# lorenzovaquero/BUSCA

Hardware: AMD Instinct MI355X
Metric: BUSCA association steps/sec (DT-step: features in HBM -> logits/probs/argmax), MOT17-like 32 lost x 16 proposals (higher is better)
Workload: dtype f32

## Files before the change

### busca_amd/csrc/busca_hip.hip

```cpp
#include "busca_internal.hpp"

#define BUSCA_DT_BUCKET_KERNEL 1
#include "dt_kernel.hip.inc"
#include "pairwise_kernel.hip.inc"
#include "track_kernel.hip.inc"
#include "crop_kernel.hip.inc"
#include "ecc_kernel.hip.inc"

int ensure_lds(busca_ctx* c, const void* kern, size_t bytes) {
    if (c->lds_configured.count(kern)) return BUSCA_OK;
    HIP_TRY(c, hipFuncSetAttribute(kern, hipFuncAttributeMaxDynamicSharedMemorySize, (int)bytes));
    c->lds_configured.insert(kern);
    return BUSCA_OK;
}

enum { OPT_INT , OPT_FLAG , OPT_PRESENT , OPT_READONLY  };
struct BuscaOptionDesc { const char* env; const char* opt; int BuscaOptions::*field; int kind; };
static const BuscaOptionDesc BUSCA_OPTIONS[] = {
    {"BUSCA_DT_NTRK", "dt_ntrk", &BuscaOptions::dt_ntrk, OPT_INT}, {"BUSCA_DT_TILED", "dt_tiled", &BuscaOptions::dt_tiled, OPT_PRESENT},
    {"BUSCA_DT_SPLIT", "dt_split", &BuscaOptions::dt_split, OPT_INT}, {"BUSCA_DT_PROF", nullptr, &BuscaOptions::dt_prof, OPT_INT},
    {"BUSCA_DT_PRUNE", "dt_prune", &BuscaOptions::dt_prune, OPT_INT}, {nullptr, "last_dt_prune", &BuscaOptions::last_dt_prune, OPT_READONLY},
    {"BUSCA_DTL_RT", nullptr, &BuscaOptions::dtl_rt, OPT_INT}, {"BUSCA_DTL_RT_MASK", nullptr, &BuscaOptions::dtl_rt_mask, OPT_INT},
    {"BUSCA_DTL_FFN", nullptr, &BuscaOptions::dtl_ffn, OPT_INT}, {"BUSCA_DTL_ATTN", nullptr, &BuscaOptions::dtl_attn, OPT_INT},
    {"BUSCA_CROP_BAND", "crop_band", &BuscaOptions::crop_band, OPT_INT}, {nullptr, "dt_exact_f32", &BuscaOptions::dt_exact_f32, OPT_FLAG},
    {nullptr, "last_dt_grid", &BuscaOptions::last_dt_grid, OPT_READONLY}, {nullptr, "last_dt_ntrk", &BuscaOptions::last_dt_ntrk, OPT_READONLY},
    {nullptr, "last_dt_split", &BuscaOptions::last_dt_split, OPT_READONLY},
    {"BUSCA_ASSIGN_STAGE", "assign_stage", &BuscaOptions::assign_stage, OPT_INT}, {nullptr, "last_assign_staged", &BuscaOptions::last_assign_staged, OPT_READONLY},
};
static const BuscaOptionDesc* option_by_name(const char* name) {
    for (const BuscaOptionDesc& e : BUSCA_OPTIONS) if (e.opt && !strcmp(e.opt, name)) return &e;
    return nullptr;
}
static void options_from_env(BuscaOptions& o) {
    for (const BuscaOptionDesc& e : BUSCA_OPTIONS)
        if (const char* t = e.env ? getenv(e.env) : nullptr) o.*e.field = e.kind == OPT_PRESENT ? 1 : atoi(t);
}

extern "C" int busca_version(void) { return 2002; }

static std::string g_create_err;

extern "C" int busca_ctx_create(int device, busca_ctx** out) {
    if (!out) return BUSCA_EINVAL;
    *out = nullptr;
    int n = 0;
    hipError_t e = hipGetDeviceCount(&n);
    if (e != hipSuccess || n <= 0) {
        g_create_err = std::string("hipGetDeviceCount: ") + hipGetErrorString(e) + ", devices=" + std::to_string(n);
        return BUSCA_EHIP;
    }
    if (device < 0 || device >= n) { g_create_err = "device index out of range"; return BUSCA_EINVAL; }
    e = hipSetDevice(device);
    if (e != hipSuccess) { g_create_err = std::string("hipSetDevice: ") + hipGetErrorString(e); return BUSCA_EHIP; }
    busca_ctx* c = new busca_ctx();
    c->device = device;
    options_from_env(c->opt);
    c->reid = reid_state_new();
    *out = c;
    return BUSCA_OK;
}

#ifndef BUSCA_BUILD_FLAGS
#define BUSCA_BUILD_FLAGS "unknown"
#endif
extern "C" const char* busca_build_info(void) { return "libbusca_hip gfx950 flags: " BUSCA_BUILD_FLAGS; }

extern "C" int busca_set_option(busca_ctx* c, const char* name, int32_t value) {
    if (!c || !name) return BUSCA_EINVAL;
    if (!strncmp(name, "reid_", 5)) return reid_set_option(c, name, value);
    if (!strcmp(name, "dt_status")) { if (c->dt.xerr) *c->dt.xerr = value; return BUSCA_OK; }
    const BuscaOptionDesc* e = option_by_name(name);
    if (!e || e->kind == OPT_READONLY) return fail(c, BUSCA_EINVAL, "busca_set_option: unknown option '%s'", name);
    c->opt.*e->field = e->kind == OPT_FLAG ? value != 0 : value;
    return BUSCA_OK;
}
extern "C" int busca_get_option(busca_ctx* c, const char* name, int32_t* value) {
    if (!c || !name || !value) return BUSCA_EINVAL;
    if (!strncmp(name, "reid_", 5)) return reid_get_option(c, name, value);
    if (!strcmp(name, "dt_status")) { *value = c->dt.xerr ? *c->dt.xerr : 0; return BUSCA_OK; }
    const BuscaOptionDesc* e = option_by_name(name);
    if (!e) return fail(c, BUSCA_EINVAL, "busca_get_option: unknown option '%s'", name);
    *value = c->opt.*e->field;
    return BUSCA_OK;
}

void timing_drain(busca_ctx* c) {
    for (auto& pr : c->ev_pending) {
        float ms = 0.f;
        if (hipEventSynchronize(pr.second) == hipSuccess && hipEventElapsedTime(&ms, pr.first, pr.second) == hipSuccess) {
            c->t_ms += ms;
            c->t_n += 1;
        }
        c->ev_free.push_back(pr.first);
        c->ev_free.push_back(pr.second);
    }
    c->ev_pending.clear();
}

extern "C" void busca_ctx_destroy(busca_ctx* c) {
    if (!c) return;
    hipSetDevice(c->device);
    hipDeviceSynchronize();
    timing_drain(c);
    for (auto e : c->ev_free) hipEventDestroy(e);
// ... 355 lines not shown
```

### busca_amd/csrc/busca_internal.hpp

```cpp
#pragma once
#include <hip/hip_runtime.h>
#include <hip/hip_fp16.h>

#include <algorithm>
#include <cmath>
#include <cstdarg>
#include <cstdio>
#include <cstdlib>
#include <cstring>
#include <set>
#include <string>
#include <type_traits>
#include <vector>

#pragma GCC visibility push(default)
#include "../../include/busca_hip.h"
#pragma GCC visibility pop
#include "dt_types.hpp"

struct ReidState;

struct DTTiledW {
    const void* w_embed = nullptr;
    const void *w_in[DT_MAX_LAYERS] = {}, *w_out[DT_MAX_LAYERS] = {}, *w1[DT_MAX_LAYERS] = {}, *w2[DT_MAX_LAYERS] = {};
};

struct DTState {
    bool loaded = false;
    busca_dt_cfg cfg{};
    void* dev_blob = nullptr;
    size_t dev_bytes = 0;
    DTParams proto{};
    void* dev_blob32 = nullptr;
    DTParams proto32{};
    void* dev_tiled = nullptr;
    DTTiledW tw;
    void* ws = nullptr; size_t ws_bytes = 0;
    void* xch = nullptr; unsigned* xflag = nullptr; float* xlg = nullptr; int* xerr = nullptr; int* xerr_dev = nullptr; int xslots = 0; unsigned xepoch = 0;
    int num_cu = 256;
};

struct BuscaOptions {
    int dt_ntrk = 0;
    int dt_tiled = 0;
    int dtl_rt = 0;
    int dtl_rt_mask = -1;
    int dtl_ffn = 2;
    int dtl_attn = 1;
    int dt_split = -1;
    int dt_prune = -1;
    int dt_prof = 0;
    int dt_exact_f32 = 0;
    int crop_band = 1;
    int assign_stage = -1;
    int last_assign_staged = 0;
    int last_dt_grid = 0, last_dt_ntrk = 0, last_dt_split = 0;
    int last_dt_prune = 0;
};

struct busca_ctx {
    int device = 0;
    std::string err;
    BuscaOptions opt;
    DTState dt;
    ReidState* reid = nullptr;
    bool timing = false;
    std::vector<std::pair<hipEvent_t, hipEvent_t>> ev_pending;
    std::vector<hipEvent_t> ev_free;
    double t_ms = 0.0;
    long long t_n = 0;
    int* crop_fill = nullptr;
    int crop_fill_cap = 0;
    std::set<const void*> lds_configured;
    void* ecc_ws = nullptr; size_t ecc_ws_bytes = 0;
};

int ensure_lds(busca_ctx* c, const void* kern, size_t bytes);

static inline int fail(busca_ctx* c, int code, const char* fmt, ...) {
    char buf[512];
    va_list ap;
    va_start(ap, fmt);
    vsnprintf(buf, sizeof buf, fmt, ap);
    va_end(ap);
    if (c) c->err = buf;
    return code;
}
#define HIP_TRY(c, call)                                                                                   \
    do {                                                                                                   \
        hipError_t e__ = (call);                                                                           \
        if (e__ != hipSuccess) return fail((c), BUSCA_EHIP, "%s -> %s", #call, hipGetErrorString(e__));     \
    } while (0)


void timing_drain(busca_ctx* c);
hipEvent_t timing_event(busca_ctx* c);
struct TimedLaunch {
    busca_ctx* c; hipStream_t s; hipEvent_t e0{}, e1{}; bool on;
    TimedLaunch(busca_ctx* c_, hipStream_t s_) : c(c_), s(s_), on(c_->timing) {
        if (on) { e0 = timing_event(c); e1 = timing_event(c); hipEventRecord(e0, s); }
    }
    ~TimedLaunch() {
        if (on) { hipEventRecord(e1, s); c->ev_pending.emplace_back(e0, e1); if (c->ev_pending.size() > 4096) timing_drain(c); }
    }
};

#define BUSCA_ENOKERNEL 1000
int dt_fused_f32(busca_ctx* c, const DTParams& K, int MT, int d, hipStream_t s);
int dt_fused_f16(busca_ctx* c, const DTParams& K, int MT, int d, bool two, hipStream_t s);
int dt_fused_x3(busca_ctx* c, const DTParams& K, int MT, int d, hipStream_t s);
int dt_tiled_f32(busca_ctx* c, const DTParams& K, int d, hipStream_t s);
int dt_tiled_f16(busca_ctx* c, const DTParams& K, int d, hipStream_t s);
int dt_tiled_x3(busca_ctx* c, const DTParams& K, int d, hipStream_t s);
int dt_split_ensure(busca_ctx* c);
size_t dtl_ws_bytes(size_t M, int D, int FF, size_t es);
int dtl_ws_ensure(busca_ctx* c, size_t need, hipStream_t s);
void dt_bucket_ids_launch(busca_ctx* c, hipStream_t s, const float* mem_ltrb, const float* can_ltrb, int B, int L, int P, int fake_f64, int can_pos, int nspec, int sep_can, int* ids);
ReidState* reid_state_new();
void reid_state_delete(ReidState* r);
bool reid_state_loaded(const ReidState* r);
int reid_set_option(busca_ctx* c, const char* name, int32_t value);
int reid_get_option(busca_ctx* c, const char* name, int32_t* value);
```

### busca_amd/csrc/dt_kernel.hip.inc

```

#pragma clang fp contract(off)

#include "dt_types.hpp"

static __device__ __forceinline__ float dt_fma(float a, float b, float c) { return __builtin_fmaf(a, b, c); }
static __device__ __forceinline__ f32x4 dt_fma(f32x4 a, f32x4 b, f32x4 c) { return __builtin_elementwise_fma(a, b, c); }

#define DT_STAMP(slot) do { if (p.prof != nullptr && blockIdx.x == 0 && lane == 0) p.prof[wave * DT_PROF_SLOTS + (slot)] = (long long)__builtin_readcyclecounter(); } while (0)

template <int PREC> struct Prec;
template <> struct Prec<0> {
    typedef float elem;
    typedef u32x4 op_t;
    static constexpr int ES = 4, EP = 4, CHUNK = 16, SUB = 4, CW = 64;
    static __device__ __forceinline__ op_t wload(const u32x4* __restrict__ w) { return *w; }
    static __device__ __forceinline__ op_t xload(const char* p, int) { return *(const u32x4*)p; }
    static __device__ __forceinline__ f32x4 unscale(f32x4 v) { return v; }
    static __device__ __forceinline__ f32x4 prescale(f32x4 v) { return v; }
    static __device__ __forceinline__ void mma(f32x4& acc, u32x4 a, u32x4 b) {
        f32x4 af = __builtin_bit_cast(f32x4, a), bf = __builtin_bit_cast(f32x4, b);
        acc = __builtin_amdgcn_mfma_f32_16x16x4f32(af[0], bf[0], acc, 0, 0, 0);
        acc = __builtin_amdgcn_mfma_f32_16x16x4f32(af[1], bf[1], acc, 0, 0, 0);
        acc = __builtin_amdgcn_mfma_f32_16x16x4f32(af[2], bf[2], acc, 0, 0, 0);
        acc = __builtin_amdgcn_mfma_f32_16x16x4f32(af[3], bf[3], acc, 0, 0, 0);
// ... 26 lines not shown
        h16x8 h;
        f32x4 lo = t[2 * c];
        f32x4 hi = (2 * c + 1 < NT) ? t[(2 * c + 1 < NT) ? 2 * c + 1 : 0] : (f32x4){0.f, 0.f, 0.f, 0.f};
#pragma unroll
        for (int r = 0; r < 4; ++r) { h[r] = (_Float16)lo[r]; h[4 + r] = (_Float16)hi[r]; }
        return __builtin_bit_cast(u32x4, h);
    }
    static __device__ __forceinline__ bool store4(char* p, f32x4 v, int = 0) {
        h16x4 h; h[0] = (_Float16)v[0]; h[1] = (_Float16)v[1]; h[2] = (_Float16)v[2]; h[3] = (_Float16)v[3];
        *(h16x4*)p = h;
        return false;
    }
    static __device__ __forceinline__ float exp(float x) { return __expf(x); }
    static __device__ __forceinline__ f32x4 gelu(f32x4 v) {
        const f32x4 s = v * 0.70710678118654752440f;
        f32x4 ax = __builtin_elementwise_min(__builtin_elementwise_abs(s), (f32x4){4.f, 4.f, 4.f, 4.f});
        auto k4 = [](float c) { return (f32x4){c, c, c, c}; };
        f32x4 q = dt_fma(ax, k4(-0.00014198364806361496f), k4(0.0036634085699915886f));
        q = dt_fma(q, ax, k4(-0.030893569812178612f));
        q = dt_fma(q, ax, k4(0.1496966928243637f));
        q = dt_fma(q, ax, k4(0.9181665182113647f));
        q = dt_fma(q, ax, k4(1.627924919128418f));
        const f32x4 m = q * -ax;
        f32x4 e;
#pragma unroll
        for (int r = 0; r < 4; ++r) e[r] = __builtin_amdgcn_exp2f(m[r]);
        f32x4 erf_ = 1.0f - e;
#pragma unroll
        for (int r = 0; r < 4; ++r) erf_[r] = __builtin_copysignf(erf_[r], s[r]);
        return (v * 0.5f) * (erf_ + 1.0f);
    }
};

struct X3Op { u32x4 hi, lo; };
typedef _Float16 dt_h16x2 __attribute__((ext_vector_type(2)));
typedef float dt_f32x2 __attribute__((ext_vector_type(2)));
static __device__ __forceinline__ void dt_split2(float t0, float t1, unsigned& hi, unsigned& lo) {
    const dt_h16x2 h = __builtin_convertvector((dt_f32x2){t0, t1}, dt_h16x2);
    hi = __builtin_bit_cast(unsigned, h);
    unsigned l;
    asm("v_fma_mixlo_f16 %0, %1, -1.0, %2 op_sel_hi:[1,0,0]" : "=v"(l) : "v"(hi), "v"(t0));
    asm("v_fma_mixhi_f16 %0, %1, -1.0, %2 op_sel:[1,0,0] op_sel_hi:[1,0,0]" : "+v"(l) : "v"(hi), "v"(t1));
    lo = l;
}
template <> struct Prec<2> {
    typedef _Float16 elem;
    typedef X3Op op_t;
    static constexpr int ES = 4, EP = 2, CHUNK = 32, SUB = 8, CW = 128;
    static __device__ __forceinline__ op_t wload(const u32x4* __restrict__ w) { op_t o; o.hi = w[0]; o.lo = w[64]; return o; }
    static __device__ __forceinline__ op_t xload(const char* p, int po) { op_t o; o.hi = *(const u32x4*)p; o.lo = *(const u32x4*)(p + po); return o; }
    static __device__ __forceinline__ void mma(f32x4& acc, op_t a, op_t b) {
        acc = __builtin_amdgcn_mfma_f32_16x16x32_f16(__builtin_bit_cast(h16x8, a.lo), __builtin_bit_cast(h16x8, b.hi), acc, 0, 0, 0);
        acc = __builtin_amdgcn_mfma_f32_16x16x32_f16(__builtin_bit_cast(h16x8, a.hi), __builtin_bit_cast(h16x8, b.lo), acc, 0, 0, 0);
        acc = __builtin_amdgcn_mfma_f32_16x16x32_f16(__builtin_bit_cast(h16x8, a.hi), __builtin_bit_cast(h16x8, b.hi), acc, 0, 0, 0);
    }
    static __device__ __forceinline__ f32x4 unscale(f32x4 v) { return v * (1.0f / (DT_X3_XS * DT_X3_WS)); }
    static __device__ __forceinline__ f32x4 prescale(f32x4 v) { return v * (DT_X3_XS * DT_X3_WS); }
    static __device__ __forceinline__ bool store4(char* p, f32x4 v, int po) {
        const f32x4 lim = {65504.f, 65504.f, 65504.f, 65504.f};
        const f32x4 sv = v * DT_X3_XS, av = __builtin_elementwise_abs(sv);
        const bool clipped = fmaxf(fmaxf(av[0], av[1]), fmaxf(av[2], av[3])) > 65504.f;
        const f32x4 s = __builtin_elementwise_min(__builtin_elementwise_max(sv, -lim), lim);
        unsigned h0, h1, l0, l1;
        dt_split2(s[0], s[1], h0, l0);
        dt_split2(s[2], s[3], h1, l1);
        *(u32x2*)p = (u32x2){h0, h1};
        *(u32x2*)(p + po) = (u32x2){l0, l1};
        return clipped;
    }
    static __device__ __forceinline__ float exp(float x) { return __expf(x); }
    static __device__ __forceinline__ f32x4 gelu(f32x4 v) { return Prec<0>::gelu(v); }
};
template <int PREC> struct AttPrec { typedef Prec<PREC == 2 ? 0 : PREC> type; };


template <int PREC, int NW, int PF, int WMAX>
__device__ __forceinline__ void gemm_prefetch(typename Prec<PREC>::op_t (&wf)[PF][WMAX], const u32x4* __restrict__ w, int tstride) {
#pragma unroll
    for (int p = 0; p < PF; ++p)
#pragma unroll
        for (int i = 0; i < NW; ++i) wf[p][i] = Prec<PREC>::wload(w + i * tstride + p * Prec<PREC>::CW);
}

template <int PREC, int NW, int NX, int NKC, int PF, bool W_IS_A, int NWN, int WMAX, int XM = 0>
__device__ __forceinline__ void gemm_stream(f32x4 (&acc)[NW][NX], typename Prec<PREC>::op_t (&wf)[PF][WMAX], const u32x4* __restrict__ w, int tstride,
                                            const char* lds, int RS, const u32x4* __restrict__ wn, int tstride_n) {
    static_assert(NKC % PF == 0 && NW <= WMAX && NWN <= WMAX && (XM != 1 || PF % 2 == 0), "bad streaming geometry");
    typedef Prec<PREC> PR;
    constexpr int CW = PR::CW;
    const int po = (RS - 16) / 2;
    typename PR::op_t xf[XM == 1 ? 2 : 1][NX];
    if constexpr (XM == 1) {
#pragma unroll
        for (int j = 0; j < NX; ++j) xf[0][j] = PR::xload(lds + j * 16 * RS, po);
    }
#pragma unroll 1
    for (int k0 = 0; k0 < NKC; k0 += PF) {
#pragma unroll
        for (int p = 0; p < PF; ++p) {
            const int kx = k0 + p + 1 < NKC ? k0 + p + 1 : NKC - 1;
            if constexpr (XM == 1) {
#pragma unroll
                for (int j = 0; j < NX; ++j) xf[(p + 1) & 1][j] = PR::xload(lds + j * 16 * RS + kx * 64, po);
                __builtin_amdgcn_sched_barrier(0);
            } else {
#pragma unroll
                for (int j = 0; j < NX; ++j) xf[0][j] = PR::xload(lds + j * 16 * RS + (k0 + p) * 64, po);
            }
            constexpr int XS = XM == 1 ? 1 : 0;
#pragma unroll
            for (int i = 0; i < NW; ++i)
#pragma unroll
                for (int j = 0; j < NX; ++j) {
                    if (W_IS_A) Prec<PREC>::mma(acc[i][j], wf[p][i], xf[p & XS][j]);
                    else        Prec<PREC>::mma(acc[i][j], xf[p & XS][j], wf[p][i]);
                }
            const int kn = k0 + p + PF;
            if (kn < NKC) {
#pragma unroll
                for (int i = 0; i < NW; ++i) wf[p][i] = PR::wload(w + i * tstride + kn * CW);
            } else if (NWN > 0) {
#pragma unroll
                for (int i = 0; i < NWN; ++i) wf[p][i] = PR::wload(wn + i * tstride_n + (kn - NKC) * CW);
            }
        }
    }
}

static __device__ __forceinline__ float xor_sum_b(float v) {
    v += __shfl_xor(v, 16);
    v += __shfl_xor(v, 32);
    return v;
}
static __device__ __forceinline__ float xor_max_b(float v) {
    v = fmaxf(v, __shfl_xor(v, 16));
    v = fmaxf(v, __shfl_xor(v, 32));
    return v;
}

template <typename R> static __device__ __forceinline__ R log_r(R x);
template <> __device__ __forceinline__ float log_r<float>(float x) { return (float)log((double)x); }
template <> __device__ __forceinline__ double log_r<double>(double x) { return log(x); }

template <typename R>
static __device__ __forceinline__ void bucket_xy_size(R x1, R y1, R x2, R y2, float rx1, float ry1, float rx2,
                                                      float ry2, int& ixy, int& isz) {
#pragma clang fp contract(off)
    const float w_ref = rx2 - rx1 + 1.f, h_ref = ry2 - ry1 + 1.f;
    const float cx_ref = 0.5f * (rx1 + rx2), cy_ref = 0.5f * (ry1 + ry2);
    const R w = x2 - x1 + (R)1, h = y2 - y1 + (R)1;
    const R cx = (R)0.5 * (x1 + x2), cy = (R)0.5 * (y1 + y2);
    R dx = (cx - (R)cx_ref) / w; dx = dx * dx;
    R dy = (cy - (R)cy_ref) / h; dy = dy * dy;
    const R eps = (R)1e-3;
    R xy = log_r<R>(sqrt(dx + dy) + eps);
    R sz = log_r<R>(w / (R)w_ref + eps) + log_r<R>(h / (R)h_ref + eps);
    xy = xy * (R)15; sz = sz * (R)15;
    xy = fmin(fmax(xy, (R)-105), (R)105);
    sz = fmin(fmax(sz, (R)-105), (R)105);
    ixy = (int)xy + 105;
    isz = (int)sz + 105;
}

static __device__ __forceinline__ void token_bucket(const float* mem_ltrb, const float* can_ltrb, int trk, int t,
                                                    int L, int P, int fake_f64, int can_pos, int nspec, int sep_can,
                                                    int& ixy, int& isz, int& it) {
    const float* ref = mem_ltrb + ((size_t)trk * L + (L - 1)) * 4;
    const float rx1 = ref[0], ry1 = ref[1], rx2 = ref[2], ry2 = ref[3];
    if (t < L) {
        const float* bx = mem_ltrb + ((size_t)trk * L + t) * 4;
        int v = (t - L + 1) * 2; v = v < -30 ? -30 : (v > 30 ? 30 : v);
        it = v + 30;
        bucket_xy_size<float>(bx[0], bx[1], bx[2], bx[3], rx1, ry1, rx2, ry2, ixy, isz);
        return;
    }
    const int k = t - L, j = k >> 1, odd = k & 1;
    it = odd ? 34 : 32;
    float x1 = rx1, y1 = ry1, x2 = rx2, y2 = ry2;
    bool fake = false;
    if (nspec == 2 && j == P + 1) fake = true;
    else if (j < P && (odd == can_pos || sep_can)) { const float* bx = can_ltrb + ((size_t)trk * P + j) * 4; x1 = bx[0]; y1 = bx[1]; x2 = bx[2]; y2 = bx[3]; }
    if (fake_f64) {
        double X1 = x1, Y1 = y1, X2 = x2, Y2 = y2;
        if (fake) { const double m = -3.4028234663852886e38; X1 = m; Y1 = m; X2 = -m / 100.0; Y2 = -m / 100.0; }
        bucket_xy_size<double>(X1, Y1, X2, Y2, rx1, ry1, rx2, ry2, ixy, isz);
    } else {
        if (fake) { const float m = -3.4028234663852886e38f; x1 = m; y1 = m; x2 = -m / 100.0f; y2 = -m / 100.0f; }
        bucket_xy_size<float>(x1, y1, x2, y2, rx1, ry1, rx2, ry2, ixy, isz);
    }
}
// ... 593 lines not shown

    if (p.hidden != nullptr) {
#pragma unroll
        for (int ft = 0; ft < NTW; ++ft)
#pragma unroll
            for (int tt = 0; tt < MTT; ++tt) {
                const int t = 16 * (tt % MTL) + a + tok0, gt = tbase + tt / MTL;
                if (t < T && gt < p.B) *(f32x4*)(p.hidden + ((size_t)gt * T + t) * D + fbase + 16 * ft + 4 * b) = X[ft][tt];
            }
    }
    {
        f32x4 dg[NTW], db[NTW];
        load_vec4<NTW>(dg, p.dec_g, fbase + 4 * b);
        load_vec4<NTW>(db, p.dec_b, fbase + 4 * b);
        layer_norm_regs<NTW, MTT>(X, dg, db, red1, red2, wave, a, b, invD);
    }
    f32x4 dw[NTW];
    load_vec4<NTW>(dw, p.dec_w, fbase + 4 * b);
#pragma unroll
    for (int tt = 0; tt < MTT; ++tt) {
        float s = 0.f;
#pragma unroll
        for (int ft = 0; ft < NTW; ++ft) {
#pragma unroll
            for (int r = 0; r < 4; ++r) s = dt_fma(X[ft][tt][r], dw[ft][r], s);
        }
        s = xor_sum_b(s);
        if (b == 0) red1[wave * TP + 16 * tt + a] = s;
    }
    __syncthreads();
    if constexpr (SPLIT) {
        const unsigned stamp = p.xepoch * 16u + 1u;
        if (wave == 0 && tile != 0) {
            if (lane < 16 * NTRK) {
                const float v = (red1[lane] + red1[TP + lane]) + (red1[2 * TP + lane] + red1[3 * TP + lane]);
                __hip_atomic_store(p.xlg + ((size_t)(xslot + lane / 16) * MT + tile) * 16 + (lane & 15), v, __ATOMIC_RELAXED, __HIP_MEMORY_SCOPE_AGENT);
            }
            DT_XFENCE_RELEASE();
            asm volatile("s_waitcnt vmcnt(0)" ::: "memory");
            if (lane < NTRK) __hip_atomic_store(p.xflag + ((size_t)(xslot + lane) * MT + tile) * DT_XFLAGS + 4, stamp, __ATOMIC_RELAXED, __HIP_MEMORY_SCOPE_AGENT);
        }
        if (wave < NTRK && tile == 0) dt_xwait<MT - 1>(p.xflag + ((size_t)(xslot + wave) * MT + 1) * DT_XFLAGS + 4, DT_XFLAGS, stamp, p.xerr);
    }
    if (wave < NTRK && tbase + wave < p.B && !(SPLIT && tile != 0)) {
        const int n = P + p.nspec;
        const size_t trk_ = (size_t)tbase + wave;
        float lg = -INFINITY;
        if (lane < n) {
            const int tg = L + 2 * lane + p.can_pos, t = prune ? lane : wave * TP1 + tg;
            if (SPLIT && tg >= TP1) lg = __hip_atomic_load(p.xlg + (size_t)(xslot + wave) * MT * 16 + tg, __ATOMIC_RELAXED, __HIP_MEMORY_SCOPE_AGENT) + p.dec_bias;
            else lg = ((red1[t] + red1[TP + t]) + (red1[2 * TP + t] + red1[3 * TP + t])) + p.dec_bias;
            p.logits[trk_ * n + lane] = lg;
        }
        float m = lg;
#pragma unroll
        for (int o = 32; o >= 1; o >>= 1) m = fmaxf(m, __shfl_xor(m, o));
        const float e = lane < n ? expf(lg - m) : 0.f;
        float sum = e;
#pragma unroll
        for (int o = 32; o >= 1; o >>= 1) sum += __shfl_xor(sum, o);
        const float pr = e / sum;
        if (p.probs != nullptr && lane < n) p.probs[trk_ * n + lane] = pr;
        float bv = lane < n ? pr : -1.f;
        int bi = lane;
#pragma unroll
        for (int o = 32; o >= 1; o >>= 1) {
            const float ov = __shfl_xor(bv, o);
            const int oi = __shfl_xor(bi, o);
            if (ov > bv || (ov == bv && oi < bi)) { bv = ov; bi = oi; }
        }
        if (p.argmax != nullptr && lane == 0) p.argmax[trk_] = bi;
    }
    if (PREC == 2 && clipped && p.xerr != nullptr) *p.xerr = 2;
    DT_STAMP(4 + 12 * DT_MAX_LAYERS);
}

#define BUSCA_DT_AUX_INSTANCES(X) X(1, 3, 512, 1024, 512, 1, 1, false) X(1, 4, 512, 1024, 512, 2, 1, false) X(1, 5, 256, 512, 512, 1, 1, false)
#ifndef BUSCA_DT_AUX_TU
#define BUSCA_DT_AUX_DECL(PR, M, DD, F, EE, NC, NT, SP) extern template __global__ void dt_fused_kernel<PR, M, DD, F, EE, NC, NT, SP>(const DTParams);
BUSCA_DT_AUX_INSTANCES(BUSCA_DT_AUX_DECL)
#undef BUSCA_DT_AUX_DECL
#endif

#pragma clang fp contract(fast)
```

### busca_amd/csrc/dt_launch.hpp

```cpp
#pragma once
#include "busca_internal.hpp"

static int dt_split_tracks(const busca_ctx* c, int B, int parts, int prec, bool can_pair, int* pair) {
    const DTState& S = c->dt;
    *pair = 1;
    if (S.xslots <= 0 || c->opt.dt_split == 0 || parts > DT_XMAX_MT) return 0;
    if (c->opt.dt_split > 0) {
        *pair = (c->opt.dt_split == 2 && can_pair) ? 2 : 1;
        return std::min(B, S.xslots / 2);
    }
    if (prec == BUSCA_PREC_F16) return 0;
    const int rem = B % S.num_cu;
    if (rem == 0 || rem + 1 > S.xslots) return 0;
    if (prec == BUSCA_PREC_F16X3) return 2 * parts * rem <= S.num_cu ? rem : 0;
    if (parts * rem <= S.num_cu) return rem;
    if (can_pair && parts * ((rem + 1) / 2) <= S.num_cu) { *pair = 2; return rem; }
    return 0;
}

static int dt_prof_report(busca_ctx* c, long long* d, int nwg, hipStream_t s) {
    HIP_TRY(c, hipStreamSynchronize(s));
    long long h[4 * DT_PROF_SLOTS];
    HIP_TRY(c, hipMemcpy(h, d, sizeof h, hipMemcpyDeviceToHost));
    HIP_TRY(c, hipFree(d));
    fprintf(stderr, "DT_PROF grid=%d:", nwg);
    for (int w = 0; w < 4; ++w) {
        fprintf(stderr, "\n w%d", w);
        for (int i = 1; i < DT_PROF_SLOTS; ++i)
            if (h[w * DT_PROF_SLOTS + i]) fprintf(stderr, " %d:%lld", i, h[w * DT_PROF_SLOTS + i] - h[w * DT_PROF_SLOTS]);
    }
    fprintf(stderr, "\n");
    return BUSCA_OK;
}

template <int PREC, int MT, int D, int FF, int NCH, int NTRK>
static int dt_launch_split(busca_ctx* c, const DTParams& P0, int nsplit, hipStream_t s) {
    typedef DTLds<PREC, 1, D, FF, 512, NCH, NTRK> LD;
    DTState& S = c->dt;
    auto kern = dt_fused_kernel<PREC, MT, D, FF, 512, NCH, NTRK, true>;
    const int nwg = ((nsplit + NTRK - 1) / NTRK) * MT;
    { int rc = dt_split_ensure(c); if (rc) return rc; }
    DTParams P = P0;
    P.prune = 0;
    P.nsingle = P.B - nsplit;
    P.xepoch = ++S.xepoch; P.xch = (unsigned long long*)S.xch; P.xflag = S.xflag; P.xlg = S.xlg; P.xerr = S.xerr_dev;
    { int rc = ensure_lds(c, (const void*)kern, LD::TOTAL); if (rc) return rc; }
    if (c->opt.dt_prof == 2) {
        HIP_TRY(c, hipMalloc((void**)&P.prof, 4 * DT_PROF_SLOTS * sizeof(long long)));
        HIP_TRY(c, hipMemset(P.prof, 0, 4 * DT_PROF_SLOTS * sizeof(long long)));
        hipLaunchKernelGGL(kern, dim3(nwg), dim3(256), LD::TOTAL, s, P);
        return dt_prof_report(c, P.prof, nwg, s);
    }
    hipLaunchKernelGGL(kern, dim3(nwg), dim3(256), LD::TOTAL, s, P);
    return BUSCA_OK;
}

template <int PREC, int MT, int D, int FF, int NCH, int NTRK = 1>
static int dt_launch(busca_ctx* c, const DTParams& P0, hipStream_t s) {
    typedef DTLds<PREC, MT, D, FF, 512, NCH, NTRK> LD;
    DTParams P = P0;
    P.prune = (PREC != 1 && NTRK == 1 && MT >= 2 && c->opt.dt_prune != 0 && P.hidden == nullptr && P.att == nullptr && P.P + P.nspec <= 16 * (MT - 1)) ? 1 : 0;
    c->opt.last_dt_prune = P.prune;
    static_assert(LD::TOTAL <= 160 * 1024, "LDS plan exceeds the 160 KiB of a CU");
    auto kern = dt_fused_kernel<PREC, MT, D, FF, 512, NCH, NTRK>;
    const int nwg = (P.B + NTRK - 1) / NTRK;
    c->opt.last_dt_grid = nwg; c->opt.last_dt_ntrk = NTRK; c->opt.last_dt_split = 0;
    if constexpr (MT >= 2 && MT <= DT_XMAX_MT && NTRK == 1) {
        constexpr bool PAIR = PREC != 1 && MT >= 3;
        if (c->dt.xslots > 0) {
            { int rc = ensure_lds(c, (const void*)dt_fused_kernel<PREC, MT, D, FF, 512, NCH, 1, true>, DTLds<PREC, 1, D, FF, 512, NCH, 1>::TOTAL); if (rc) return rc; }
            if constexpr (PAIR) { int rc = ensure_lds(c, (const void*)dt_fused_kernel<PREC, MT, D, FF, 512, NCH, 2, true>, DTLds<PREC, 1, D, FF, 512, NCH, 2>::TOTAL); if (rc) return rc; }
        }
        { int rc = ensure_lds(c, (const void*)kern, LD::TOTAL); if (rc) return rc; }
        int pair = 1;
        const int nsplit = c->opt.dt_prof == 1 ? 0 : dt_split_tracks(c, P.B, MT, PREC, PAIR, &pair);
        if (nsplit > 0) {
            c->opt.last_dt_grid = P.B - nsplit + ((nsplit + pair - 1) / pair) * MT; c->opt.last_dt_split = nsplit; c->opt.last_dt_ntrk = pair;
            if (P.B == nsplit) c->opt.last_dt_prune = 0;
            TimedLaunch tl(c, s);
            if (P.B > nsplit) hipLaunchKernelGGL(kern, dim3(P.B - nsplit), dim3(256), LD::TOTAL, s, P);
            int rc = BUSCA_OK;
            if constexpr (PAIR) { if (pair == 2) rc = dt_launch_split<PREC, MT, D, FF, NCH, 2>(c, P, nsplit, s); else rc = dt_launch_split<PREC, MT, D, FF, NCH, 1>(c, P, nsplit, s); }
            else rc = dt_launch_split<PREC, MT, D, FF, NCH, 1>(c, P, nsplit, s);
            if (rc) return rc;
            HIP_TRY(c, hipGetLastError());
            return BUSCA_OK;
        }
    }
    { int rc = ensure_lds(c, (const void*)kern, LD::TOTAL); if (rc) return rc; }
    const bool prof = c->opt.dt_prof == 1;
    if (prof) {
        DTParams Q = P;
        long long* d = nullptr;
        HIP_TRY(c, hipMalloc((void**)&d, 4 * DT_PROF_SLOTS * sizeof(long long)));
        HIP_TRY(c, hipMemset(d, 0, 4 * DT_PROF_SLOTS * sizeof(long long)));
        Q.prof = d;
        hipLaunchKernelGGL(kern, dim3(nwg), dim3(256), LD::TOTAL, s, Q);
        return dt_prof_report(c, d, nwg, s);
    }
    {
        TimedLaunch tl(c, s);
        hipLaunchKernelGGL(kern, dim3(nwg), dim3(256), LD::TOTAL, s, P);
    }
    HIP_TRY(c, hipGetLastError());
    return BUSCA_OK;
}
```

Baseline: 15180.

## Add unique-row DT kernel that deduplicates repeated tokens to shrink token tiles

Adds a fused DT kernel that processes only unique token rows (NU = MT-1 tiles) instead of the full padded token sequence. K/V are gathered via an index table (koff) so that duplicated separator or padding tokens map back onto shared rows. The kernel is enabled by default when the sequence fits in MT-1 tiles and no separate candidate, hidden-state or attention output is requested. This cuts embedding and Q/FFN GEMM work and LDS footprint per track, at the cost of a new code path with complex row mapping that may diverge numerically or mishandle edge cases.

After: 18310, median of 6. 20.6% higher.

```diff
diff --git a/busca_amd/csrc/busca_hip.hip b/busca_amd/csrc/busca_hip.hip
--- a/busca_amd/csrc/busca_hip.hip
+++ b/busca_amd/csrc/busca_hip.hip
@@ -20,6 +20,7 @@
     {"BUSCA_DT_NTRK", "dt_ntrk", &BuscaOptions::dt_ntrk, OPT_INT}, {"BUSCA_DT_TILED", "dt_tiled", &BuscaOptions::dt_tiled, OPT_PRESENT},
     {"BUSCA_DT_SPLIT", "dt_split", &BuscaOptions::dt_split, OPT_INT}, {"BUSCA_DT_PROF", nullptr, &BuscaOptions::dt_prof, OPT_INT},
     {"BUSCA_DT_PRUNE", "dt_prune", &BuscaOptions::dt_prune, OPT_INT}, {nullptr, "last_dt_prune", &BuscaOptions::last_dt_prune, OPT_READONLY},
+    {"BUSCA_DT_UNIQUE", "dt_unique", &BuscaOptions::dt_unique, OPT_INT}, {nullptr, "last_dt_unique", &BuscaOptions::last_dt_unique, OPT_READONLY},
     {"BUSCA_DTL_RT", nullptr, &BuscaOptions::dtl_rt, OPT_INT}, {"BUSCA_DTL_RT_MASK", nullptr, &BuscaOptions::dtl_rt_mask, OPT_INT},
     {"BUSCA_DTL_FFN", nullptr, &BuscaOptions::dtl_ffn, OPT_INT}, {"BUSCA_DTL_ATTN", nullptr, &BuscaOptions::dtl_attn, OPT_INT},
     {"BUSCA_CROP_BAND", "crop_band", &BuscaOptions::crop_band, OPT_INT}, {nullptr, "dt_exact_f32", &BuscaOptions::dt_exact_f32, OPT_FLAG},
diff --git a/busca_amd/csrc/busca_internal.hpp b/busca_amd/csrc/busca_internal.hpp
--- a/busca_amd/csrc/busca_internal.hpp
+++ b/busca_amd/csrc/busca_internal.hpp
@@ -49,12 +49,14 @@
     int dtl_attn = 1;
     int dt_split = -1;
     int dt_prune = -1;
+    int dt_unique = -1;
     int dt_prof = 0;
     int dt_exact_f32 = 0;
     int crop_band = 1;
     int assign_stage = -1;
     int last_assign_staged = 0;
     int last_dt_grid = 0, last_dt_ntrk = 0, last_dt_split = 0;
+    int last_dt_unique = 0;
     int last_dt_prune = 0;
 };
 
diff --git a/busca_amd/csrc/dt_kernel.hip.inc b/busca_amd/csrc/dt_kernel.hip.inc
--- a/busca_amd/csrc/dt_kernel.hip.inc
+++ b/busca_amd/csrc/dt_kernel.hip.inc
@@ -132,17 +132,18 @@
         for (int i = 0; i < NW; ++i) wf[p][i] = Prec<PREC>::wload(w + i * tstride + p * Prec<PREC>::CW);
 }
 
-template <int PREC, int NW, int NX, int NKC, int PF, bool W_IS_A, int NWN, int WMAX, int XM = 0>
+template <int PREC, int NW, int NX, int NKC, int PF, bool W_IS_A, int NWN, int WMAX, int XM = 0, bool XT = false>
 __device__ __forceinline__ void gemm_stream(f32x4 (&acc)[NW][NX], typename Prec<PREC>::op_t (&wf)[PF][WMAX], const u32x4* __restrict__ w, int tstride,
-                                            const char* lds, int RS, const u32x4* __restrict__ wn, int tstride_n) {
+                                            const char* lds, int RS, const u32x4* __restrict__ wn, int tstride_n, const int* xt = nullptr) {
     static_assert(NKC % PF == 0 && NW <= WMAX && NWN <= WMAX && (XM != 1 || PF % 2 == 0), "bad streaming geometry");
     typedef Prec<PREC> PR;
     constexpr int CW = PR::CW;
     const int po = (RS - 16) / 2;
     typename PR::op_t xf[XM == 1 ? 2 : 1][NX];
+    auto xrow = [&](int j) { if constexpr (XT) return xt[j]; else return j * 16 * RS; };
     if constexpr (XM == 1) {
 #pragma unroll
-        for (int j = 0; j < NX; ++j) xf[0][j] = PR::xload(lds + j * 16 * RS, po);
+        for (int j = 0; j < NX; ++j) xf[0][j] = PR::xload(lds + xrow(j), po);
     }
 #pragma unroll 1
     for (int k0 = 0; k0 < NKC; k0 += PF) {
@@ -151,11 +152,11 @@
             const int kx = k0 + p + 1 < NKC ? k0 + p + 1 : NKC - 1;
             if constexpr (XM == 1) {
 #pragma unroll
-                for (int j = 0; j < NX; ++j) xf[(p + 1) & 1][j] = PR::xload(lds + j * 16 * RS + kx * 64, po);
+                for (int j = 0; j < NX; ++j) xf[(p + 1) & 1][j] = PR::xload(lds + xrow(j) + kx * 64, po);
                 __builtin_amdgcn_sched_barrier(0);
             } else {
 #pragma unroll
-                for (int j = 0; j < NX; ++j) xf[0][j] = PR::xload(lds + j * 16 * RS + (k0 + p) * 64, po);
+                for (int j = 0; j < NX; ++j) xf[0][j] = PR::xload(lds + xrow(j) + (k0 + p) * 64, po);
             }
             constexpr int XS = XM == 1 ? 1 : 0;
 #pragma unroll
@@ -915,4 +916,6 @@
 #undef BUSCA_DT_AUX_DECL
 #endif
 
+#include "dt_unique_kernel.hip.inc"
+
 #pragma clang fp contract(fast)
diff --git a/busca_amd/csrc/dt_launch.hpp b/busca_amd/csrc/dt_launch.hpp
--- a/busca_amd/csrc/dt_launch.hpp
+++ b/busca_amd/csrc/dt_launch.hpp
@@ -63,6 +63,13 @@
     c->opt.last_dt_prune = P.prune;
     static_assert(LD::TOTAL <= 160 * 1024, "LDS plan exceeds the 160 KiB of a CU");
     auto kern = dt_fused_kernel<PREC, MT, D, FF, 512, NCH, NTRK>;
+    size_t lds_bytes = LD::TOTAL;
+    bool uniq = false;
+    if constexpr (PREC != 1 && NTRK == 1 && MT >= 2) {
+        uniq = c->opt.dt_unique != 0 && P.sep_can == 0 && P.hidden == nullptr && P.att == nullptr && P.T - P.P <= 16 * (MT - 1);
+        if (uniq) { kern = dt_fused_unique_kernel<PREC, MT, D, FF, 512, NCH>; lds_bytes = DTLds<PREC, MT - 1, D, FF, 512, NCH, 1>::TOTAL; }
+    }
+    c->opt.last_dt_unique = uniq ? 1 : 0;
     const int nwg = (P.B + NTRK - 1) / NTRK;
     c->opt.last_dt_grid = nwg; c->opt.last_dt_ntrk = NTRK; c->opt.last_dt_split = 0;
     if constexpr (MT >= 2 && MT <= DT_XMAX_MT && NTRK == 1) {
@@ -71,14 +78,14 @@
             { int rc = ensure_lds(c, (const void*)dt_fused_kernel<PREC, MT, D, FF, 512, NCH, 1, true>, DTLds<PREC, 1, D, FF, 512, NCH, 1>::TOTAL); if (rc) return rc; }
             if constexpr (PAIR) { int rc = ensure_lds(c, (const void*)dt_fused_kernel<PREC, MT, D, FF, 512, NCH, 2, true>, DTLds<PREC, 1, D, FF, 512, NCH, 2>::TOTAL); if (rc) return rc; }
         }
-        { int rc = ensure_lds(c, (const void*)kern, LD::TOTAL); if (rc) return rc; }
+        { int rc = ensure_lds(c, (const void*)kern, lds_bytes); if (rc) return rc; }
         int pair = 1;
         const int nsplit = c->opt.dt_prof == 1 ? 0 : dt_split_tracks(c, P.B, MT, PREC, PAIR, &pair);
         if (nsplit > 0) {
             c->opt.last_dt_grid = P.B - nsplit + ((nsplit + pair - 1) / pair) * MT; c->opt.last_dt_split = nsplit; c->opt.last_dt_ntrk = pair;
-            if (P.B == nsplit) c->opt.last_dt_prune = 0;
+            if (P.B == nsplit) { c->opt.last_dt_prune = 0; c->opt.last_dt_unique = 0; }
             TimedLaunch tl(c, s);
-            if (P.B > nsplit) hipLaunchKernelGGL(kern, dim3(P.B - nsplit), dim3(256), LD::TOTAL, s, P);
+            if (P.B > nsplit) hipLaunchKernelGGL(kern, dim3(P.B - nsplit), dim3(256), lds_bytes, s, P);
             int rc = BUSCA_OK;
             if constexpr (PAIR) { if (pair == 2) rc = dt_launch_split<PREC, MT, D, FF, NCH, 2>(c, P, nsplit, s); else rc = dt_launch_split<PREC, MT, D, FF, NCH, 1>(c, P, nsplit, s); }
             else rc = dt_launch_split<PREC, MT, D, FF, NCH, 1>(c, P, nsplit, s);
@@ -87,7 +94,7 @@
             return BUSCA_OK;
         }
     }
-    { int rc = ensure_lds(c, (const void*)kern, LD::TOTAL); if (rc) return rc; }
+    { int rc = ensure_lds(c, (const void*)kern, lds_bytes); if (rc) return rc; }
     const bool prof = c->opt.dt_prof == 1;
     if (prof) {
         DTParams Q = P;
@@ -95,12 +102,12 @@
         HIP_TRY(c, hipMalloc((void**)&d, 4 * DT_PROF_SLOTS * sizeof(long long)));
         HIP_TRY(c, hipMemset(d, 0, 4 * DT_PROF_SLOTS * sizeof(long long)));
         Q.prof = d;
-        hipLaunchKernelGGL(kern, dim3(nwg), dim3(256), LD::TOTAL, s, Q);
+        hipLaunchKernelGGL(kern, dim3(nwg), dim3(256), lds_bytes, s, Q);
         return dt_prof_report(c, d, nwg, s);
     }
     {
         TimedLaunch tl(c, s);
-        hipLaunchKernelGGL(kern, dim3(nwg), dim3(256), LD::TOTAL, s, P);
+        hipLaunchKernelGGL(kern, dim3(nwg), dim3(256), lds_bytes, s, P);
     }
     HIP_TRY(c, hipGetLastError());
     return BUSCA_OK;
diff --git a/busca_amd/csrc/dt_unique_kernel.hip.inc b/busca_amd/csrc/dt_unique_kernel.hip.inc
--- /dev/null
+++ b/busca_amd/csrc/dt_unique_kernel.hip.inc
@@ -0,0 +1,295 @@
+template <int PREC, int MT, int D, int FF, int E, int NCHUNK_FF>
+__global__ void __launch_bounds__(256, 1) dt_fused_unique_kernel(const DTParams p) {
+    typedef Prec<PREC> PR;
+    typedef typename AttPrec<PREC>::type APR;
+    static_assert(PREC != 1 && MT >= 2, "unique rows: the f32 / x3 flavours of two token tiles or more");
+    constexpr int NU = MT - 1;
+    constexpr int NTRK = 1, MTL = MT;
+    constexpr bool SPLIT = MT < 0, TWO = MT < 0;
+    typedef DTLds<PREC, NU, D, FF, E, NCHUNK_FF, 1> LD;
+    constexpr int EP = PR::EP, CHUNK = PR::CHUNK, CW = PR::CW;
+    constexpr int TP = 16 * NU;
+    constexpr int HD = D / 4, NTW = D / 64, FT = HD / 16;
+    constexpr int KC_D = D / CHUNK, KC_E = E / CHUNK, KC_FFC = LD::FFC / CHUNK, KC_FF = FF / CHUNK;
+    constexpr int FTW = LD::FFC / 64;
+    constexpr int WMAX = NTW > 4 ? 8 : 4;
+    constexpr int QNW = FT;
+    constexpr int FSUB = FTW > WMAX ? WMAX : FTW;
+    constexpr int RSP = D * 4 + 16;
+    constexpr int NSUB = FTW / FSUB;
+    constexpr int XM = (PREC != 0 && D == 256 && MT <= 3) ? 1 : 0;
+    constexpr int PF = PREC == 2 ? 2 : (WMAX == 8 ? 2 : (KC_D >= 4 ? 4 : KC_D));
+    constexpr int NCF = APR::nchunks(FT), NCK = APR::nchunks(MT);
+    static_assert(FT == NTW && FTW % FSUB == 0 && KC_E % PF == 0 && KC_FFC % PF == 0, "geometry");
+    static_assert(16 * NU * RSP <= LD::HB_BYTES, "pruned layer: the parked residual does not fit HB");
+
+    extern __shared__ __attribute__((aligned(16))) char smem[];
+    char* xop = smem + LD::OFF_XOP;
+    char* hb = smem + LD::OFF_HB;
+    float* red1 = (float*)(smem + LD::OFF_RED1);
+    float* red2 = (float*)(smem + LD::OFF_RED2);
+    int* ids = (int*)(smem + LD::OFF_IDS);
+
+    const int trk = blockIdx.x;
+    const int tile = 0, xslot = 0, tok0 = 0;
+    auto track_of = [&](int) { return trk; };
+    auto park_x = [&]() {};
+    const int tid = threadIdx.x;
+    const int lane = tid & 63;
+    const int wave = __builtin_amdgcn_readfirstlane(tid >> 6);
+    const int a = lane & 15, b = lane >> 4;
+    const int L = p.L, P = p.P, T = p.T;
+    const int n = P + p.nspec, U = T - P;
+    const int fbase = wave * (D / 4);
+    const bool prune = p.prune != 0;
+
+    auto tok_of = [&](int u) {
+        if (u < n) return L + 2 * u + p.can_pos;
+        if (u < n + L) return u - n;
+        if (u == n + L) return L + 2 * P + 1 - p.can_pos;
+        if (u == n + L + 1 && p.nspec == 2) return L + 2 * (P + 1) + 1 - p.can_pos;
+        return T;
+    };
+    auto row_of = [&](int t) {
+        if (t >= T) return U < TP ? U : TP - 1;
+        if (t < L) return n + t;
+        const int k = t - L, j = k >> 1;
+        if ((k & 1) == p.can_pos) return j;
+        return (p.nspec == 2 && j == P + 1) ? n + L + 1 : n + L;
+    };
+
+    const u32x4* w_emb = p.w_embed + (size_t)(wave * NTW) * KC_E * CW + lane;
+    auto wq_of = [&](const DTLayerW& W, int part) { return W.w_in + (size_t)((part * D + wave * HD) / 16) * KC_D * CW + lane; };
+
+    typename PR::op_t wf[PF][WMAX];
+    bool clipped = false;
+    DT_STAMP(0);
+    gemm_prefetch<PREC, NTW, PF, WMAX>(wf, w_emb, KC_E * CW);
+
+    if (tid < TP) {
+        int ixy = 0, isz = 0, it = 0;
+        const int t = tok_of(tid);
+        if (t < T) token_bucket(p.mem_ltrb, p.can_ltrb, trk, t, L, P, p.fake_f64, p.can_pos, p.nspec, p.sep_can, ixy, isz, it);
+        ids[tid] = ixy; ids[TP + tid] = isz; ids[2 * TP + tid] = it;
+    }
+    {
+        constexpr int NPC = TP * (E / 4) / 256;
+        constexpr int NB = NPC > 24 ? NPC / 2 : NPC;
+        static_assert(NPC % NB == 0, "staging batches");
+#pragma unroll
+        for (int q0 = 0; q0 < NPC; q0 += NB) {
+            f32x4 v[NB];
+#pragma unroll
+            for (int q = 0; q < NB; ++q) {
+                const int i = tid + 256 * (q0 + q);
+                const int row = i / (E / 4), e4 = i % (E / 4);
+                const int t = tok_of(row);
+                const int k = t - L, j = k >> 1;
+                const bool is_mem = t < L, is_can = !is_mem && t < T && (k & 1) == p.can_pos && j < P;
+                const float* src = is_can ? p.can_feat + ((size_t)trk * P + j) * E + e4 * 4 : p.mem_feat + ((size_t)trk * L + (is_mem ? t : 0)) * E + e4 * 4;
+                const f32x4 ld = *(const f32x4*)src;
+                v[q] = ld * ((is_mem || is_can) ? 1.0f : 0.0f);
+            }
+            __builtin_amdgcn_sched_barrier(0);
+#pragma unroll
+            for (int q = 0; q < NB; ++q) {
+                const int i = tid + 256 * (q0 + q);
+                clipped |= PR::store4(hb + (i / (E / 4)) * LD::RSE + (i % (E / 4)) * 4 * EP, v[q], (LD::RSE - 16) / 2);
+            }
+        }
+    }
+    __syncthreads();
+    DT_STAMP(1);
+
+    f32x4 X[NTW][NU];
+    {
+#pragma unroll
+        for (int ft = 0; ft < NTW; ++ft)
+#pragma unroll
+            for (int tt = 0; tt < NU; ++tt) X[ft][tt] = (f32x4){0.f, 0.f, 0.f, 0.f};
+        gemm_stream<PREC, NTW, NU, KC_E, PF, true, QNW, WMAX, XM>(X, wf, w_emb, KC_E * CW, hb + a * LD::RSE + b * 16, LD::RSE, wq_of(p.layer[0], 1), KC_D * CW);
+        DT_STAMP(2);
+        const float sq = sqrtf((float)D);
+        const int c = p.lut_c;
+#pragma unroll
+        for (int tt = 0; tt < NU; ++tt) {
+            const int row = 16 * tt + a;
+            const int t = tok_of(row);
+            int kind;
+            if (t >= T) kind = 4;
+            else if (t < L) kind = 0;
+            else { const int k = t - L, j = k >> 1; kind = (k & 1) == p.can_pos ? (j < P ? 0 : (j == P ? 2 : 3)) : 1; }
+            const _Float16* rxy = p.lut_xy + ids[row] * c;
+            const _Float16* rsz = p.lut_sz + ids[TP + row] * c - c;
+            const _Float16* rt = p.lut_t + ids[2 * TP + row] * c - 2 * c;
+            const float* tokv = kind == 2 ? p.tok_non : (kind == 3 ? p.tok_bad : p.tok_sep);
+#pragma unroll
+            for (int ft = 0; ft < NTW; ++ft) {
+                const int f0 = fbase + 16 * ft + 4 * b;
+                const f32x4 be = *(const f32x4*)(p.b_embed + f0);
+                const f32x4 tk = *(const f32x4*)(tokv + f0);
+                const f32x4 xu = PR::unscale(X[ft][tt]);
+                f32x4 enc;
+#pragma unroll
+                for (int r = 0; r < 4; ++r) {
+                    const int f = f0 + r;
+                    const _Float16* src = f < c ? rxy : (f < 2 * c ? rsz : rt);
+                    enc[r] = (float)src[f];
+                }
+#pragma unroll
+                for (int r = 0; r < 4; ++r) {
+                    const float base = kind == 0 ? (xu[r] + be[r]) * sq : tk[r];
+                    X[ft][tt][r] = kind == 4 ? 0.f : base + enc[r];
+                }
+            }
+        }
+    }
+    clipped |= store_rows<PREC, NTW, NU>(X, xop, LD::RSX, a, b, fbase);
+    __syncthreads();
+    DT_STAMP(3);
+
+    const float invD = 1.0f / (float)D;
+    const float qscale = 1.0f / sqrtf((float)HD);
+    int koff[MT];
+#pragma unroll
+    for (int i = 0; i < MT; ++i) koff[i] = row_of(16 * i + a) * LD::RSX;
+
+#pragma unroll 1
+    for (int l = 0; l < p.nlayers; ++l) {
+        const DTLayerW& W = p.layer[l];
+        const DTLayerW& Wn = p.layer[l + 1 < p.nlayers ? l + 1 : l];
+        const u32x4* w_out = W.w_out + (size_t)(wave * NTW) * KC_D * CW + lane;
+        const int sl = 4 + 12 * l;
+        u32x4 qf[NU][NCF], kf[MT][NCF], vf[1][FT][NCK];
+        f32x4 kown[1][FT], vown[1][FT];
+        constexpr size_t XW = 0; const unsigned xstamp = 0;
+        const char* xl = xop + a * LD::RSX + b * 16;
+        const f32x4 zero4 = {0.f, 0.f, 0.f, 0.f};
+        {
+            f32x4 acc[FT][MT];
+            f32x4 bk[FT]; float bv[FT];
+            load_vec4<FT>(bk, W.b_in, D + wave * HD + 4 * b);
+#pragma unroll
+            for (int ft = 0; ft < FT; ++ft)
+#pragma unroll
+                for (int tt = 0; tt < MT; ++tt) acc[ft][tt] = zero4;
+            gemm_stream<PREC, FT, MT, KC_D, PF, true, FT, WMAX, XM, true>(acc, wf, wq_of(W, 1), KC_D * CW, xop + b * 16, LD::RSX, wq_of(W, 2), KC_D * CW, koff);
+            DT_STAMP(sl + 0);
+#pragma unroll
+            for (int tt = 0; tt < MT; ++tt) {
+                f32x4 tl[FT];
+#pragma unroll
+                for (int ft = 0; ft < FT; ++ft) tl[ft] = PR::unscale(acc[ft][tt]) + bk[ft];
+#pragma unroll
+                for (int c = 0; c < NCF; ++c) kf[tt][c] = APR::template frag<FT>(tl, c);
+            }
+#pragma unroll
+            for (int ft = 0; ft < FT; ++ft) bv[ft] = W.b_in[2 * D + wave * HD + 16 * ft + a];
+#pragma unroll
+            for (int ft = 0; ft < FT; ++ft)
+#pragma unroll
+                for (int tt = 0; tt < MT; ++tt) acc[ft][tt] = zero4;
+            gemm_stream<PREC, FT, MT, KC_D, PF, false, FT, WMAX, XM, true>(acc, wf, wq_of(W, 2), KC_D * CW, xop + b * 16, LD::RSX, wq_of(W, 0), KC_D * CW, koff);
+            DT_STAMP(sl + 1);
+#pragma unroll
+            for (int ft = 0; ft < FT; ++ft) {
+                f32x4 tl[MT];
+#pragma unroll
+                for (int tt = 0; tt < MT; ++tt) tl[tt] = PR::unscale(acc[ft][tt]) + bv[ft];
+#pragma unroll
+                for (int c = 0; c < NCK; ++c) vf[0][ft][c] = APR::template frag<MT>(tl, c);
+            }
+        }
+        if (prune && l == p.nlayers - 1) {
+#pragma unroll
+            for (int ft = 0; ft < NTW; ++ft)
+#pragma unroll
+                for (int tt = 0; tt < NU; ++tt) *(f32x4*)(hb + (16 * tt + a) * RSP + (fbase + 16 * ft + 4 * b) * 4) = X[ft][tt];
+            __syncthreads();
+#pragma unroll
+            for (int tt = 0; tt < NU; ++tt) {
+                const int r = 16 * tt + a < n ? 16 * tt + a : n - 1;
+#pragma unroll
+                for (int ft = 0; ft < NTW; ++ft) X[ft][tt] = *(const f32x4*)(hb + r * RSP + (fbase + 16 * ft + 4 * b) * 4);
+            }
+            clipped |= store_rows<PREC, NTW, NU>(X, xop, LD::RSX, a, b, fbase);
+            __syncthreads();
+        }
+        {
+            f32x4 acc[FT][NU];
+            f32x4 bq[FT];
+            load_vec4<FT>(bq, W.b_in, wave * HD + 4 * b);
+#pragma unroll
+            for (int ft = 0; ft < FT; ++ft)
+#pragma unroll
+                for (int tt = 0; tt < NU; ++tt) acc[ft][tt] = zero4;
+            gemm_stream<PREC, FT, NU, KC_D, PF, true, NTW, WMAX, XM>(acc, wf, wq_of(W, 0), KC_D * CW, xl, LD::RSX, w_out, KC_D * CW);
+            DT_STAMP(sl + 2);
+#pragma unroll
+            for (int tt = 0; tt < NU; ++tt) {
+                f32x4 tl[FT];
+#pragma unroll
+                for (int ft = 0; ft < FT; ++ft) tl[ft] = (PR::unscale(acc[ft][tt]) + bq[ft]) * qscale;
+#pragma unroll
+                for (int c = 0; c < NCF; ++c) qf[tt][c] = APR::template frag<FT>(tl, c);
+            }
+        }
+#define DT_NQL NU
+#define DT_NQT NU
+#define DT_XQ X
+#define DT_KNEXT true
+#include "dt_layer_tail.hip.inc"
+#undef DT_NQL
+#undef DT_NQT
+#undef DT_XQ
+#undef DT_KNEXT
+    }
+
+    {
+        f32x4 dg[NTW], db[NTW];
+        load_vec4<NTW>(dg, p.dec_g, fbase + 4 * b);
+        load_vec4<NTW>(db, p.dec_b, fbase + 4 * b);
+        layer_norm_regs<NTW, NU>(X, dg, db, red1, red2, wave, a, b, invD);
+    }
+    f32x4 dw[NTW];
+    load_vec4<NTW>(dw, p.dec_w, fbase + 4 * b);
+#pragma unroll
+    for (int tt = 0; tt < NU; ++tt) {
+        float s = 0.f;
+#pragma unroll
+        for (int ft = 0; ft < NTW; ++ft) {
+#pragma unroll
+            for (int r = 0; r < 4; ++r) s = dt_fma(X[ft][tt][r], dw[ft][r], s);
+        }
+        s = xor_sum_b(s);
+        if (b == 0) red1[wave * TP + 16 * tt + a] = s;
+    }
+    __syncthreads();
+    if (wave == 0) {
+        float lg = -INFINITY;
+        if (lane < n) {
+            lg = ((red1[lane] + red1[TP + lane]) + (red1[2 * TP + lane] + red1[3 * TP + lane])) + p.dec_bias;
+            p.logits[(size_t)trk * n + lane] = lg;
+        }
+        float m = lg;
+#pragma unroll
+        for (int o = 32; o >= 1; o >>= 1) m = fmaxf(m, __shfl_xor(m, o));
+        const float e = lane < n ? expf(lg - m) : 0.f;
+        float sum = e;
+#pragma unroll
+        for (int o = 32; o >= 1; o >>= 1) sum += __shfl_xor(sum, o);
+        const float pr = e / sum;
+        if (p.probs != nullptr && lane < n) p.probs[(size_t)trk * n + lane] = pr;
+        float bv = lane < n ? pr : -1.f;
+        int bi = lane;
+#pragma unroll
+        for (int o = 32; o >= 1; o >>= 1) {
+            const float ov = __shfl_xor(bv, o);
+            const int oi = __shfl_xor(bi, o);
+            if (ov > bv || (ov == bv && oi < bi)) { bv = ov; bi = oi; }
+        }
+        if (p.argmax != nullptr && lane == 0) p.argmax[trk] = bi;
+    }
+    if (PREC == 2 && clipped && p.xerr != nullptr) *p.xerr = 2;
+    DT_STAMP(4 + 12 * DT_MAX_LAYERS);
+}
```
